# KorAP/Datok

Measured on AMD Instinct MI355X. Metric: input MB/s tokenized, tokenizer_de.matok, higher is better.
Workload: dtype u32 table cells, u8 symbol codes; 1 GPU; tokenizer_de.matok, 4096 equal-length 4096 B synthetic German docs per batch (BASELINE.json configs[1]); table_layout=matrix: state-major fused u32 cells, docs_per_gpu=4096, doc_bytes=4096, parallelism=documents sharded over 1 GPU(s), no data-path collective, batches_in_flight=3, inputs=one per batch in flight (generator seeds 2, 3, 4 on rank 0)

## Files before the change

### datok_amd/_lib.py

```python
import ctypes as C
import os
import subprocess

_HERE = os.path.dirname(os.path.abspath(__file__))
LIB_PATH = os.environ.get("DATOK_GPU_LIB") or os.path.join(_HERE, "libdatok_gpu.so")

OK, E_IO, E_FORMAT, E_NO_DEVICE, E_HIP, E_ARG, E_MODEL, E_CAPACITY, E_STATE, E_NOMEM = 0, -1, -2, -3, -4, -5, -6, -7, -8, -9
ST_WINDOW_OVERFLOW, ST_EMPTY_TEXT, ST_BAD_MODEL, ST_IRREGULAR, ST_STEP_LIMIT, ST_INTERNAL = 1, 2, 4, 8, 16, 32
ST_BAD_OFFSET = 64

EXPORTS = [
    "dtk_device_count", "dtk_set_device", "dtk_strerror", "dtk_last_hip_error",
    "dtk_model_load", "dtk_model_load_mem", "dtk_model_free", "dtk_model_type", "dtk_model_get_info",
    "dtk_model_info_mem",
    "dtk_batch_create", "dtk_batch_free", "dtk_batch_set_input", "dtk_batch_set_input_device",
    "dtk_batch_run", "dtk_batch_sync", "dtk_batch_stream", "dtk_batch_totals",
    "dtk_batch_set_profiling", "dtk_batch_stage_ms", "dtk_batch_set_chunking", "dtk_batch_set_warm_extend",
    "dtk_batch_result_device", "dtk_batch_result_host", "dtk_transduce", "dtk_free",
    "dtk_foma_to_matok", "dtk_foma_to_datok", "dtk_transduce_replay", "dtk_batch_render_device", "dtk_batch_render_host",
    "dtk_batch_status_host", "dtk_transduce_release", "dtk_transduce_result",
    "dtk_pipeline_create", "dtk_pipeline_free", "dtk_pipeline_set_chunking", "dtk_pipeline_run",
    "dtk_pinned_alloc", "dtk_pinned_free",
    "dtk_batch_set_result_fields", "dtk_batch_download_begin", "dtk_pipeline_set_result_fields",
    "dtk_batch_set_download_stream", "dtk_batch_download_stream", "dtk_batch_done", "dtk_batch_set_streams",
    "dtk_debug_configure",
    "dtk_multi_create", "dtk_multi_free", "dtk_multi_type", "dtk_multi_set_result_fields", "dtk_multi_set_chunking", "dtk_multi_run",
]


class ModelInfo(C.Structure):
    _fields_ = [("kind", C.c_int32), ("epsilon", C.c_int32), ("unknown", C.c_int32),
                ("identity", C.c_int32), ("final_state", C.c_int32), ("sigma_count", C.c_int32),
                ("state_count", C.c_uint32), ("array_len", C.c_uint64),
                ("n_eps_states", C.c_uint32), ("max_eps_chain", C.c_uint32),
                ("entry_bytes", C.c_uint32), ("device_bytes", C.c_uint64),
                ("unknown_used", C.c_uint32), ("dense_states", C.c_uint32),
                ("stream_codes", C.c_uint32)]


class Totals(C.Structure):
    _fields_ = [("n_docs", C.c_uint32), ("n_bytes", C.c_uint64), ("n_tokens", C.c_uint64),
                ("n_sent", C.c_uint64), ("n_texts", C.c_uint64), ("n_flagged", C.c_uint64),
                ("walk_steps", C.c_uint64), ("n_lanes", C.c_uint32), ("chunk_bytes", C.c_uint32),
                ("repair_rounds", C.c_uint32)]


class ResultView(C.Structure):
    _fields_ = [("tok_off", C.c_void_p), ("sent_off", C.c_void_p), ("text_off", C.c_void_p),
                ("tok_rstart", C.c_void_p), ("tok_rend", C.c_void_p),
                ("tok_bstart", C.c_void_p), ("tok_bend", C.c_void_p),
                ("sent", C.c_void_p), ("text_tok_end", C.c_void_p), ("text_sent_end", C.c_void_p),
                ("status", C.c_void_p), ("ev_bits", C.c_void_p), ("ev_words", C.c_uint64), ("doc_tail", C.c_void_p),
                ("n_exact", C.c_uint32), ("exact_doc", C.c_void_p), ("exact_off", C.c_void_p),
                ("calls", C.c_void_p), ("tok_r16", C.c_void_p)]


SLICE_FN = C.CFUNCTYPE(C.c_int, C.c_void_p, C.c_uint32, C.c_uint32, C.c_void_p)

# ... 75 lines not shown
    L.dtk_batch_download_stream.restype = vp
    L.dtk_pipeline_set_result_fields.argtypes = [vp, u32]
    L.dtk_transduce.argtypes = [vp, C.c_char_p, sz, u32, C.POINTER(vp), C.POINTER(sz), C.POINTER(u32)]
    L.dtk_transduce_replay.argtypes = L.dtk_transduce.argtypes
    L.dtk_transduce_release.restype = None
    L.dtk_transduce_result.argtypes = [vp, C.c_char_p, sz, u32, C.POINTER(ResultView)]
    L.dtk_batch_render_device.argtypes = [vp, u32, C.POINTER(RenderView)]
    L.dtk_batch_render_host.argtypes = [vp, u32, C.POINTER(RenderView)]
    L.dtk_batch_status_host.argtypes = [vp, vp, u32]
    L.dtk_foma_to_matok.argtypes = [vp, C.c_size_t, C.POINTER(vp), C.POINTER(C.c_size_t)]
    L.dtk_foma_to_matok.restype = C.c_int
    L.dtk_foma_to_datok.argtypes = [vp, C.c_size_t, C.POINTER(vp), C.POINTER(C.c_size_t)]
    L.dtk_foma_to_datok.restype = C.c_int
    L.dtk_free.argtypes = [vp]
    L.dtk_free.restype = None
    L.dtk_pipeline_create.argtypes = [u64, u32, u32, C.POINTER(vp)]
    L.dtk_pipeline_free.argtypes = [vp]
    L.dtk_pipeline_free.restype = None
    L.dtk_pipeline_set_chunking.argtypes = [vp, u32, u32]
    L.dtk_pipeline_run.argtypes = [vp, vp, vp, vp, u32, u32, SLICE_FN, vp]
    L.dtk_multi_create.argtypes = [C.c_char_p, C.POINTER(C.c_int), u32, u64, u32, u32, C.POINTER(vp)]
    L.dtk_multi_free.argtypes = [vp]
    L.dtk_multi_free.restype = None
    L.dtk_multi_type.argtypes = [vp]
    L.dtk_multi_type.restype = C.c_char_p
    L.dtk_multi_set_result_fields.argtypes = [vp, u32]
    L.dtk_multi_set_chunking.argtypes = [vp, u32, u32]
    L.dtk_multi_run.argtypes = [vp, vp, vp, u32, u32, SLICE_FN, vp]
    L.dtk_pinned_alloc.restype = vp
    L.dtk_pinned_alloc.argtypes = [sz]
    L.dtk_pinned_free.argtypes = [vp]
    L.dtk_pinned_free.restype = None
    L.dtk_debug_configure.argtypes = [C.c_char_p, C.c_char_p]
    for k, v in os.environ.items():
        if k.startswith("DATOK_") and k not in ("DATOK_GPU_LIB", "DATOK_GATHER_TIMEOUT"):
            L.dtk_debug_configure(k.encode(), v.encode())
    _lib = L
    return L


def check(code, what=""):
    if code != OK:
        raise DatokGpuError(code, what)
```

### datok_amd/csrc/dtk_batch.cpp

```cpp
#include <algorithm>
#include <cstdio>
#include <cstring>

#include "dtk_host.h"

int pin_fit(dtk_batch::PinBuf &pb, size_t n) {
  if (n <= pb.cap && pb.p) return DTK_OK;
  if (pb.p) HIP_TRY(hipHostFree(pb.p));
  pb.p = nullptr; pb.cap = 0;
  const size_t cap = std::max<size_t>(n + n / 4, 256);
  HIP_TRY(hipHostMalloc(&pb.p, cap, hipHostMallocDefault));
  pb.cap = cap;
  return DTK_OK;
}

static int alloc_outputs(dtk_batch *b, uint64_t tok, uint64_t sent, uint64_t text) {
  auto grow = [&](auto *&p, uint64_t n) -> int {
    if (p) HIP_TRY(hipFree(p));
    p = nullptr;
    HIP_TRY(hipMalloc((void **)&p, std::max<uint64_t>(n, 4) * 4));
    return DTK_OK;
  };
  int rc;
  if (tok > b->tok_cap) {
// ... 401 lines not shown
  b->repair_rounds = 0;
  hipStream_t s = b->stream;
  const bool prof = b->profiling;
#define STAGE(i) do { if (prof) HIP_TRY(hipEventRecord(b->ev[i], s)); } while (0)
  STAGE(0);
  bool fold_acc = false;
  size_t acc_bytes = 0;
  {
    const size_t nd = b->n_docs;
    uint8_t *q = b->d_acc;
    b->d_tok_off = b->d_csr; b->d_sent_off = b->d_csr + (nd + 1); b->d_text_off = b->d_csr + 2 * (nd + 1);
    b->d_totals = (uint64_t *)q; q += DTK_TOTALS_BYTES;
    b->d_tok_cnt = (uint64_t *)q; q += (nd + 1) * 8;
    b->d_sent_cnt = (uint64_t *)q; q += (nd + 1) * 8;
    b->d_text_cnt = (uint64_t *)q; q += (nd + 1) * 8;
    b->d_status = (uint32_t *)q; q += nd * 4;
    b->d_first_bad = (uint32_t *)q; q += nd * 4;
    b->d_fail_lane = (uint32_t *)q; q += nd * 4;
    b->d_doc_tail = (uint32_t *)q; q += nd * 4;
    const size_t acc_used = ((size_t)(q - b->d_acc) + 15) & ~(size_t)15;
    b->bit_words = (uint32_t)(((b->total + nd) / 32 + 8) & ~(uint64_t)3);
    const bool fold = b->total > 0;
    fold_acc = fold && b->acc_primed && acc_used / 16 < 0xFFFFFFFFull && !g_dbg.clear_kernel;
    if (!fold_acc) {
      if (dtk_launch_clear2(b->d_acc, acc_used, b->d_bits, fold ? 0 : (size_t)EVB_KINDS * b->bit_words * 4, s))
        return hip_fail(hipGetLastError(), "clear");
      b->acc_primed = true;
    }
    acc_bytes = acc_used;
  }
  STAGE(1);
  if (dtk_launch_symbolize(b->d_text, b->d_off, b->n_docs, b->total, &m->sig, b->d_sym,
                           b->d_text == b->d_text_own, b->d_blk_doc, (unsigned long long *)(b->d_totals + 6), b->d_rsbits,
                           b->d_bits, b->bit_words, fold_acc ? b->d_acc : nullptr, acc_bytes, ++b->epoch, s))
    return hip_fail(hipGetLastError(), "symbolize");
  STAGE(2);
  DtkWalkArgs w = walk_args(b);
  bool fix_in_scan = false;
  DtkSpecArgs sp_first{};
  if (b->chunk == 0) {
    STAGE(3); STAGE(4);
    if (dtk_launch_walk(&m->tab, &w, s)) return hip_fail(hipGetLastError(), "walk");
    STAGE(5); STAGE(6); STAGE(7);
  } else {
    DtkSpecArgs sp = spec_args(b, false);
    sp_first = sp;
    uint32_t *nb = (uint32_t *)(b->d_totals + 8);
    const bool split = g_dbg.split_start != 0 || sp.lds_words == 0;
    b->dev_rounds = g_dbg.dev_rounds >= 0 ? (uint32_t)g_dbg.dev_rounds : (b->expect_repairs ? 2u : 0u);
    if (b->dev_rounds > 3u) b->dev_rounds = 3u;
    fix_in_scan = b->n_docs <= 8192u && b->dev_rounds == 0;
#define SPEC(stage)                                                                               \
  do {                                                                                            \
    if (dtk_launch_spec(&m->tab, &w, &sp, stage, cmp_mask_of(m), b->d_redo, nb, s))               \
      return hip_fail(hipGetLastError(), "speculative walk");                                     \
  } while (0)
    if (split) {
      SPEC(0); STAGE(3); SPEC(1); STAGE(4); SPEC(2); STAGE(5); SPEC(3); STAGE(6);
    } else {
      STAGE(3); STAGE(4); SPEC(6); STAGE(5); SPEC(7); STAGE(6);
    }
    if (!fix_in_scan) SPEC(4);
    STAGE(7);
#undef SPEC
    for (uint32_t r = 0; r < b->dev_rounds; r++) {
      DtkSpecArgs rp = spec_args(b, true);
      rp.go = nb + r;
// ... 248 lines not shown
```

### datok_amd/csrc/dtk_host.h

```cpp
#pragma once
#include <hip/hip_runtime.h>

#include <string>
#include <type_traits>
#include <vector>

#include "../../include/datok_gpu.h"
#include "dtk_internal.h"

#pragma GCC visibility push(hidden)


int hip_fail(hipError_t e, const char *what);
#define HIP_TRY(call)                                   \
  do {                                                  \
    hipError_t e_ = (call);                             \
    if (e_ != hipSuccess) return hip_fail(e_, #call);   \
  } while (0)

struct DtkDebug {
  int sym16 = 0;
  int force_wide = 0;
  int file_columns = 0;
  int no_fused = 0;
  int wide_fused = 0;
  int no_dense = 0;
  int small_max = -1;
  int lds_bits = 1;
  int split_start = 0;
  int dev_rounds = -1;
  int compact_full = 0;
  int clear_kernel = 0;
  int round_limit = -1;
  int debug_repair = 0;
};
extern DtkDebug g_dbg;


struct dtk_model {
  int kind = 0;
  int epsilon = 0, unknown = 0, identity = 0, final_state = 0, sigma_count = 0;
  uint32_t state_count = 0;
  std::vector<uint16_t> col;
  uint32_t dense_states = 0;
  uint64_t array_len = 0;
  uint32_t n_eps_states = 0, max_eps_chain = 0, unknown_used = 0;
  uint64_t device_bytes = 0;
  int device = 0;
  bool host_only = false;
  std::vector<uint32_t> sigma_runes;
  std::vector<uint16_t> sigma_syms;
  uint16_t ascii[256];
  void *d_tab = nullptr;
  uint16_t *d_ascii = nullptr;
  uint32_t *d_runes = nullptr;
  uint16_t *d_syms = nullptr;
  void *d_codes = nullptr;
  DtkTableDev tab{};
  DtkSigmaDev sig{};
// ... 146 lines not shown
```

### datok_amd/csrc/dtk_internal.h

```cpp
#pragma once
#include <stddef.h>
#include <stdint.h>

#define DTK_FIRSTBIT 0x80000000u
#define DTK_SECONDBIT 0x40000000u
#define DTK_RESTBIT 0x3fffffffu
#define DTK_EOT 4u
#define DTK_WINDOW 1024u
#define DTK_WINDOW_BYTES 4104u

#define DTK_SYM_MASK 0x7FFu
#define DTK_SYM_MAX 2047u
#define DTK_SYM_W_SHIFT 11
#define DTK_SYM_CLS_SHIFT 14
#define DTK_SYM_WIDTH(e) (((uint32_t)(e) >> DTK_SYM_W_SHIFT) & 7u)
#define DTK_SYM_IS_START(e) (DTK_SYM_WIDTH(e) != 0u)
#define DTK_WIN 32u
#define DTK_WIN_ROW 36u
#define DTK_SYM_CONT 0xFFu
#ifndef DTK_WIN8
#define DTK_WIN8 32u
#endif
struct DtkSym {
  const void *base;
// ... 203 lines not shown
  const uint32_t *doc_ns;
  struct DtkSym sym;
  uint64_t *A, *P, *Q;
  uint64_t *blkA, *blkP, *blkQ;
  uint64_t *ns_off;
  uint64_t *tx_base, *tx_stream, *tx_pos, *tx_sent;
  uint64_t *out_off;
  uint8_t *out;
  uint64_t out_total;
};

#define DTK_TOHOST_MAX 14
struct DtkToHostArgs {
  const void *src[DTK_TOHOST_MAX];
  void *dst[DTK_TOHOST_MAX];
  uint64_t bytes[DTK_TOHOST_MAX];
  int32_t count_from[DTK_TOHOST_MAX];
  uint64_t cap[DTK_TOHOST_MAX];
  uint32_t n;
  const uint64_t *totals;
  const uint32_t *skip_if;
  uint64_t *done;
  uint64_t epoch;
};

#ifdef __cplusplus
extern "C" {
#endif
int dtk_launch_to_host(const struct DtkToHostArgs *args, void *stream);
int dtk_launch_pack_r16(const int32_t *rs, const int32_t *re, uint32_t *out, uint64_t n, void *stream);
int dtk_launch_symbolize(const uint8_t *text, const uint64_t *doc_off, uint32_t n_docs,
                         uint64_t total, const struct DtkSigmaDev *sig, void *sym, int padded,
                         const uint32_t *blk_doc, unsigned long long *n_invalid, uint32_t *rs_bits,
                         uint32_t *ev_bits, uint32_t bit_words, void *acc, uint64_t acc_bytes, uint64_t epoch, void *stream);
#ifndef DTK_SYM_BLOCK_BYTES
#define DTK_SYM_BLOCK_BYTES 4096u
#endif
int dtk_launch_walk(const struct DtkTableDev *tab, const struct DtkWalkArgs *args, void *stream);
int dtk_launch_spec(const struct DtkTableDev *tab, const struct DtkWalkArgs *args,
                    const struct DtkSpecArgs *spec, int stage, uint32_t cmp_mask, uint32_t *redo_out,
                    uint32_t *n_bad, void *stream);
int dtk_launch_spec_check(const struct DtkWalkArgs *args, const struct DtkSpecArgs *spec, int stage, uint32_t cmp_mask,
                          uint32_t *redo_out, uint32_t *n_bad, void *stream);
int dtk_launch_redo_clear(const struct DtkWalkArgs *args, const struct DtkSpecArgs *spec, void *stream);
int dtk_launch_compact(const struct DtkCompactArgs *args, uint32_t small_max, const uint32_t *big_docs, uint32_t n_big,
                       int which, void *stream);
int dtk_launch_exact(const struct DtkTableDev *tab, const struct DtkExactArgs *args, void *stream);
int dtk_launch_seg_prepare(const struct DtkCompactArgs *args, const uint32_t *doc_seg0, void *stream);
int dtk_launch_render(const struct DtkRenderArgs *args, int stage, void *stream);
uint32_t dtk_render_tiles(uint64_t n);
int dtk_launch_clear2(void *a, uint64_t a_bytes, void *b, uint64_t b_bytes, void *stream);
int dtk_launch_scan3(const uint64_t *ca, const uint64_t *cb, const uint64_t *cc, uint64_t *a, uint64_t *b,
                     uint64_t *c, uint32_t n_docs, uint64_t *totals, const uint32_t *status, uint64_t *ws,
                     const struct DtkSpecArgs *fix_spec, uint32_t *redo_out, uint32_t *n_bad, const uint32_t *skip_if,
                     void *stream);
#ifdef __cplusplus
}
#endif
```

### datok_amd/csrc/dtk_model.cpp

```cpp
#include <zlib.h>

#include <algorithm>
#include <cstdio>
#include <cstdlib>
#include <cstring>

#include "dtk_host.h"


static thread_local std::string g_hip_err;

int hip_fail(hipError_t e, const char *what) {
  g_hip_err = std::string(what) + ": " + hipGetErrorString(e);
  return e == hipErrorNoDevice || e == hipErrorInvalidDevice ? DTK_E_NO_DEVICE : DTK_E_HIP;
}

extern "C" const char *dtk_last_hip_error(void) { return g_hip_err.c_str(); }

extern "C" const char *dtk_strerror(int code) {
  switch (code) {
    case DTK_OK: return "ok";
    case DTK_E_IO: return "cannot open or read the tokenizer file";
    case DTK_E_FORMAT: return "not a gzip'd MATOK/DATOK file (magic, version or length)";
    case DTK_E_NO_DEVICE: return "no usable HIP device (this library has no CPU path)";
    case DTK_E_HIP: return "HIP runtime error (see dtk_last_hip_error)";
    case DTK_E_ARG: return "invalid argument";
    case DTK_E_MODEL: return "model outside device limits (symbols >= 2048, special ids out of range, epsilon cycle)";
    case DTK_E_CAPACITY: return "batch exceeds the capacity it was created with";
    case DTK_E_STATE: return "call out of order";
    case DTK_E_NOMEM: return "out of host memory";
    default: return "unknown error";
  }
}

extern "C" int dtk_device_count(void) {
  int n = 0;
  if (hipGetDeviceCount(&n) != hipSuccess) return 0;
  return n;
}

extern "C" int dtk_set_device(int device) {
  HIP_TRY(hipSetDevice(device));
  return DTK_OK;
}

DtkDebug g_dbg;

extern "C" int dtk_debug_configure(const char *key, const char *value) {
  if (!key) return DTK_E_ARG;
  const int v = value ? atoi(value) : 1;
  const struct { const char *name; int *field; bool flag; } tab[] = {
      {"SYM16", &g_dbg.sym16, true}, {"FORCE_WIDE", &g_dbg.force_wide, true}, {"FILE_COLUMNS", &g_dbg.file_columns, true},
      {"NO_FUSED", &g_dbg.no_fused, true}, {"WIDE_FUSED", &g_dbg.wide_fused, true}, {"NO_DENSE", &g_dbg.no_dense, true}, {"SMALL_MAX", &g_dbg.small_max, false},
      {"LDS_BITS", &g_dbg.lds_bits, false}, {"SPLIT_START", &g_dbg.split_start, false}, {"DEV_ROUNDS", &g_dbg.dev_rounds, false},
      {"COMPACT_FULL", &g_dbg.compact_full, true}, {"CLEAR_KERNEL", &g_dbg.clear_kernel, true},
      {"ROUND_LIMIT", &g_dbg.round_limit, false}, {"DEBUG_REPAIR", &g_dbg.debug_repair, true}};
  if (strncmp(key, "DATOK_", 6) == 0) key += 6;
  for (const auto &e : tab)
    if (strcmp(key, e.name) == 0) {
      *e.field = e.flag ? ((value && value[0] == '0' && value[1] == 0) ? 0 : 1) : v;
      return DTK_OK;
    }
  return DTK_E_ARG;
}


int go_decode_host(const uint8_t *p, size_t n, uint32_t *r) {
  *r = 0xFFFD;
  if (n == 0) return 0;
  uint32_t b0 = p[0];
  if (b0 < 0x80) { *r = b0; return 1; }
  if (b0 < 0xC2 || b0 > 0xF4) return 1;
  if (b0 < 0xE0) {
    if (n < 2 || (p[1] & 0xC0) != 0x80) return 1;
    *r = ((b0 & 0x1F) << 6) | (p[1] & 0x3F);
    return 2;
  }
  if (b0 < 0xF0) {
    uint32_t lo = b0 == 0xE0 ? 0xA0 : 0x80, hi = b0 == 0xED ? 0x9F : 0xBF;
    if (n < 3 || p[1] < lo || p[1] > hi || (p[2] & 0xC0) != 0x80) return 1;
    *r = ((b0 & 0x0F) << 12) | ((uint32_t)(p[1] & 0x3F) << 6) | (p[2] & 0x3F);
    return 3;
  }
  uint32_t lo = b0 == 0xF0 ? 0x90 : 0x80, hi = b0 == 0xF4 ? 0x8F : 0xBF;
  if (n < 4 || p[1] < lo || p[1] > hi || (p[2] & 0xC0) != 0x80 || (p[3] & 0xC0) != 0x80) return 1;
  *r = ((b0 & 0x07) << 18) | ((uint32_t)(p[1] & 0x3F) << 12) | ((uint32_t)(p[2] & 0x3F) << 6) | (p[3] & 0x3F);
// ... 508 lines not shown
```

### datok_amd/csrc/dtk_symbolize.hip

```cpp
#include "dtk_device.h"


__device__ __forceinline__ uint32_t go_width(uint32_t b0, uint32_t b1, uint32_t b2, uint32_t b3, uint32_t avail) {
  const uint32_t c1 = (b1 & 0xC0u) == 0x80u, c2 = (b2 & 0xC0u) == 0x80u, c3 = (b3 & 0xC0u) == 0x80u;
  const uint32_t two = (uint32_t)(b0 - 0xC2u < 0x1Eu) & (uint32_t)(avail >= 2u) & c1;
  const uint32_t lo3 = b0 == 0xE0u ? 0xA0u : 0x80u, hi3 = b0 == 0xEDu ? 0x9Fu : 0xBFu;
  const uint32_t three = (uint32_t)((b0 & 0xF0u) == 0xE0u) & (uint32_t)(avail >= 3u) & (uint32_t)(b1 >= lo3) &
                         (uint32_t)(b1 <= hi3) & c2;
  const uint32_t lo4 = b0 == 0xF0u ? 0x90u : 0x80u, hi4 = b0 == 0xF4u ? 0x8Fu : 0xBFu;
  const uint32_t four = (uint32_t)(b0 - 0xF0u <= 4u) & (uint32_t)(avail >= 4u) & (uint32_t)(b1 >= lo4) &
                        (uint32_t)(b1 <= hi4) & c2 & c3;
  return 1u + two + 2u * three + 3u * four;
}


#define SYM_BLOCK_BYTES DTK_SYM_BLOCK_BYTES
#define SYM_TILE 512u
#define SYM_SIG_LDS 64u
#define SYM_HALF 1024u
#define SYM_THREADS (WAVE * (SYM_BLOCK_BYTES / SYM_HALF))
#define SYM_DOFF (SYM_BLOCK_BYTES / 16u)

template <bool ALIGNED4, bool SYM8>
__global__ __launch_bounds__(SYM_THREADS) void k_symbolize(const uint8_t *__restrict__ text,
                                                    const uint64_t *__restrict__ doc_off,
                                                    uint32_t n_docs, uint64_t total, DtkSigmaDev sig,
                                                    void *__restrict__ sym_,
                                                    const uint32_t *__restrict__ blk_doc,
                                                    unsigned long long *__restrict__ n_invalid,
                                                    uint32_t *__restrict__ rs_bits,
                                                    uint32_t *__restrict__ ev_bits, uint32_t bit_words,
                                                    uint4 *__restrict__ acc, uint32_t acc16,
                                                    unsigned long long epoch) {
  if (acc) {
    const uint4 z = make_uint4(0u, 0u, 0u, 0u);
    for (uint32_t i = blockIdx.x * SYM_THREADS + threadIdx.x; i < acc16; i += gridDim.x * SYM_THREADS) {
      if (i == 3u) reinterpret_cast<unsigned long long *>(acc)[7] = 0ull;
      else acc[i] = z;
    }
  }
  uint16_t *__restrict__ sym = static_cast<uint16_t *>(sym_);
  uint8_t *__restrict__ sym8 = static_cast<uint8_t *>(sym_);
  __shared__ uint32_t s_rs[SYM_BLOCK_BYTES / 32];
  __shared__ uint16_t lut[128];
  __shared__ uint16_t lat[256];
  __shared__ uint32_t s_runes[SYM_SIG_LDS];
  __shared__ uint16_t s_syms[SYM_SIG_LDS];
  __shared__ uint32_t s_txt[SYM_BLOCK_BYTES / 4 + 4];
  __shared__ uint16_t s_qs[SYM_BLOCK_BYTES / SYM_HALF][SYM_HALF];
  __shared__ uint64_t s_doff[SYM_DOFF];
  const uint32_t tid = threadIdx.x, lane = tid & (WAVE - 1u), half = tid >> 6;
  uint16_t *s_q = s_qs[half];
  const bool sig_lds = sig.n_runes <= SYM_SIG_LDS;
  for (uint32_t i = tid; i < SYM_BLOCK_BYTES / 32; i += SYM_THREADS) s_rs[i] = 0;
  for (uint32_t i = tid; i < 256u; i += SYM_THREADS) {
    if (SYM8) {
      lat[i] = sig.code_lt256[i];
      if (sig_lds && i < sig.n_runes) { s_runes[i] = sig.runes[i]; s_syms[i] = sig.code_runes[i]; }
    } else {
      const uint32_t e = (sig.ascii[i] & DTK_SYM_MASK) | (i == DTK_EOT ? (1u << DTK_SYM_CLS_SHIFT) : 0u);
      lat[i] = (uint16_t)e;
      if (i < 128u) lut[i] = (uint16_t)(e | (1u << DTK_SYM_W_SHIFT));
      if (sig_lds && i < sig.n_runes) { s_runes[i] = sig.runes[i]; s_syms[i] = sig.syms[i]; }
    }
  }
  const uint64_t block_start = (uint64_t)blockIdx.x * SYM_BLOCK_BYTES;
  const uint32_t n_here = (uint32_t)min((uint64_t)SYM_BLOCK_BYTES, total - block_start);
  const uint32_t d_lo = blk_doc[blockIdx.x];
  const uint32_t d_hi = min(blk_doc[blockIdx.x + 1], n_docs - 1);
  const uint32_t n_off = d_hi - d_lo + 2u;
  if (n_off <= SYM_DOFF && tid < n_off) s_doff[tid] = doc_off[d_lo + tid];
  {
    auto load4 = [&](uint64_t g) -> uint32_t {
      if (ALIGNED4) return g < total ? *reinterpret_cast<const uint32_t *>(text + g) : 0u;
      uint32_t x = 0;
      for (int k = 0; k < 4; k++)
        if (g + k < total) x |= (uint32_t)text[g + k] << (8 * k);
      return x;
    };
    uint32_t v[SYM_BLOCK_BYTES / 4 / SYM_THREADS];
#pragma unroll
    for (uint32_t r = 0; r < SYM_BLOCK_BYTES / 4 / SYM_THREADS; r++) v[r] = load4(block_start + (r * SYM_THREADS + tid) * 4u);
    uint32_t halo = 0;
    if (tid == 0 && block_start >= 4) halo = load4(block_start - 4);
    if (tid == 1) halo = load4(block_start + SYM_BLOCK_BYTES);
#pragma unroll
    for (uint32_t r = 0; r < SYM_BLOCK_BYTES / 4 / SYM_THREADS; r++) s_txt[1 + r * SYM_THREADS + tid] = v[r];
    if (tid == 0) s_txt[0] = halo;
    if (tid == 1) s_txt[1 + SYM_BLOCK_BYTES / 4] = halo;
  }
  __syncthreads();
  const uint8_t *__restrict__ sb = reinterpret_cast<const uint8_t *>(s_txt) + 4;

  const uint64_t lo_start = doc_off[d_lo], lo_end = doc_off[d_lo + 1];
  if (ev_bits) {
    const uint64_t ga = block_start + d_lo, gb = block_start + n_here + d_hi + 1u;
    const uint32_t wa = blockIdx.x == 0 ? 0u : (uint32_t)(ga >> 5);
    uint32_t wb = (uint32_t)((gb + 31u) >> 5);
    if (wb > bit_words || blockIdx.x == gridDim.x - 1) wb = bit_words;
    for (uint32_t w = wa + tid; w < wb; w += SYM_THREADS)
#pragma unroll
      for (uint32_t k = 0; k < EVB_KINDS; k++) ev_bits[(size_t)k * bit_words + w] = 0u;
  }
  const bool sym16 = ((reinterpret_cast<uintptr_t>(sym_) + (SYM8 ? 1ull : 2ull) * block_start) & (SYM8 ? 7u : 15u)) == 0;

  if (half * SYM_HALF < n_here) {
    uint32_t qn = 0;
    auto light = [&](auto full_tag, uint32_t it) {
      constexpr bool FULL = decltype(full_tag)::value;
      const uint32_t i0 = half * SYM_HALF + it * SYM_TILE + lane * 8u;
      const uint32_t w0 = s_txt[1 + (i0 >> 2)], w1 = s_txt[2 + (i0 >> 2)];
      uint32_t left = 8u;
      if (!FULL) left = i0 < n_here ? (n_here - i0 >= 8u ? 8u : n_here - i0) : 0u;
      if (SYM8) {
        if (FULL || (left == 8u && sym16)) {
          *reinterpret_cast<uint2 *>(sym8 + block_start + i0) = make_uint2(w0, w1);
        } else {
          for (uint32_t j = 0; j < left; j++) sym8[block_start + i0 + j] = (uint8_t)((j < 4u ? w0 >> (8u * j) : w1 >> (8u * j - 32u)));
        }
      } else {
        const uint32_t e0 = lut[w0 & 0x7Fu], e1 = lut[(w0 >> 8) & 0x7Fu];
        const uint32_t e2 = lut[(w0 >> 16) & 0x7Fu], e3 = lut[(w0 >> 24) & 0x7Fu];
        const uint32_t e4 = lut[w1 & 0x7Fu], e5 = lut[(w1 >> 8) & 0x7Fu];
        const uint32_t e6 = lut[(w1 >> 16) & 0x7Fu], e7 = lut[(w1 >> 24) & 0x7Fu];
        if (FULL || (left == 8u && sym16)) {
          *reinterpret_cast<uint4 *>(sym + block_start + i0) =
              make_uint4(e0 | (e1 << 16), e2 | (e3 << 16), e4 | (e5 << 16), e6 | (e7 << 16));
        } else {
          const uint32_t o[8] = {e0, e1, e2, e3, e4, e5, e6, e7};
          for (uint32_t j = 0; j < left; j++) sym[block_start + i0 + j] = (uint16_t)o[j];
        }
      }
      auto nib = [](uint32_t x) { return ((x >> 7) & 1u) | ((x >> 14) & 2u) | ((x >> 21) & 4u) | ((x >> 28) & 8u); };
      const uint32_t valid = FULL ? 0xFFu : ((1u << left) - 1u);
      const uint32_t rare = (nib(w0 & 0x80808080u) | (nib(w1 & 0x80808080u) << 4)) & valid;
      const uint32_t asc = ~rare & valid;
// ... 75 lines not shown
            const int m = (l + h) >> 1;
            const uint32_t r = sig_lds ? s_runes[m] : sig.runes[m];
            if (r == rune) {
              if (SYM8)
                a_cls = wd == 1u ? (uint32_t)sig.code_fffd1 : (sig_lds ? (uint32_t)s_syms[m] : (uint32_t)sig.code_runes[m]);
              else
                a_cls = ((sig_lds ? (uint32_t)s_syms[m] : (uint32_t)sig.syms[m]) & DTK_SYM_MASK) |
                        (2u << DTK_SYM_CLS_SHIFT);
              break;
            }
            if (r < rune) l = m + 1; else h = m - 1;
          }
        }
        if (SYM8) sym8[g] = (uint8_t)(start ? a_cls : DTK_SYM_CONT);
        else sym[g] = (uint16_t)(a_cls | (start ? wd << DTK_SYM_W_SHIFT : 0u));
        if (start) atomicOr(&s_rs[pos >> 5], 1u << (pos & 31u));
        bad = start && wd == 1u;
      }
      if (__ballot(bad) != 0ull && lane == 0 &&
          __hip_atomic_load(n_invalid, __ATOMIC_RELAXED, __HIP_MEMORY_SCOPE_AGENT) != epoch)
        atomicMax(n_invalid, epoch);
    }
  }
  __syncthreads();
  for (uint32_t i = tid; i < SYM_BLOCK_BYTES / 32; i += SYM_THREADS)
    if (i * 32u < n_here) rs_bits[(block_start >> 5) + i] = s_rs[i];
}


extern "C" int dtk_launch_symbolize(const uint8_t *text, const uint64_t *doc_off, uint32_t n_docs,
                                    uint64_t total, const DtkSigmaDev *sig, void *sym, int padded,
                                    const uint32_t *blk_doc, unsigned long long *n_invalid, uint32_t *rs_bits,
                                    uint32_t *ev_bits, uint32_t bit_words, void *acc, uint64_t acc_bytes,
                                    uint64_t epoch, void *stream) {
  if (total == 0 || n_docs == 0) return 0;
  const uint32_t blocks = (uint32_t)((total + SYM_BLOCK_BYTES - 1) / SYM_BLOCK_BYTES);
  const bool al4 = (((uintptr_t)text) & 3u) == 0 && (padded || (total & 3u) == 0);
  auto go = [&](auto k) {
    hipLaunchKernelGGL(k, dim3(blocks), dim3(SYM_THREADS), 0, (hipStream_t)stream, text, doc_off, n_docs,
                       total, *sig, sym, blk_doc, n_invalid, rs_bits, ev_bits, bit_words, (uint4 *)acc, (uint32_t)(acc_bytes / 16),
                       (unsigned long long)epoch);
  };
  if (sig->n_codes) { if (al4) go(k_symbolize<true, true>); else go(k_symbolize<false, true>); }
  else { if (al4) go(k_symbolize<true, false>); else go(k_symbolize<false, false>); }
  return (int)hipGetLastError();
}
```

### include/datok_gpu.h

```cpp
#ifndef DATOK_GPU_H
#define DATOK_GPU_H

#include <stddef.h>
#include <stdint.h>

#ifdef __cplusplus
extern "C" {
#endif

enum {
  DTK_OK = 0,
  DTK_E_IO = -1,
  DTK_E_FORMAT = -2,
  DTK_E_NO_DEVICE = -3,
  DTK_E_HIP = -4,
  DTK_E_ARG = -5,
  DTK_E_MODEL = -6,
  DTK_E_CAPACITY = -7,
  DTK_E_STATE = -8,
  DTK_E_NOMEM = -9
};

enum {
  DTK_TOKENS = 1,
  DTK_SENTENCES = 2,
  DTK_TOKEN_POS = 4,
  DTK_SENTENCE_POS = 8,
  DTK_NEWLINE_AFTER_EOT = 16,
  DTK_SIMPLE = 3,
  DTK_OFFSETS_ONLY = 256,
  DTK_NO_BYTE_OFFSETS = 512,
  DTK_NO_RUNE_OFFSETS = 1024
};

enum {
  DTK_ST_WINDOW_OVERFLOW = 1,
  DTK_ST_EMPTY_TEXT = 2,
  DTK_ST_BAD_MODEL = 4,
  DTK_ST_IRREGULAR = 8,
  DTK_ST_STEP_LIMIT = 16,
  DTK_ST_INTERNAL = 32,
  DTK_ST_BAD_OFFSET = 64
};

typedef struct dtk_model dtk_model;
typedef struct dtk_batch dtk_batch;

int dtk_device_count(void);
int dtk_set_device(int device);
const char *dtk_strerror(int code);
const char *dtk_last_hip_error(void);

int dtk_debug_configure(const char *key, const char *value);

int dtk_model_load(const char *path, dtk_model **out);
int dtk_model_load_mem(const void *gz_bytes, size_t n, dtk_model **out);
void dtk_model_free(dtk_model *m);
int dtk_foma_to_matok(const void *gz_bytes, size_t n, void **out, size_t *out_n);
int dtk_foma_to_datok(const void *gz_bytes, size_t n, void **out, size_t *out_n);
const char *dtk_model_type(const dtk_model *m);

typedef struct {
  int32_t kind;
  int32_t epsilon, unknown, identity, final_state, sigma_count;
  uint32_t state_count;
  uint64_t array_len;
  uint32_t n_eps_states;
  uint32_t max_eps_chain;
  uint32_t entry_bytes;
  uint64_t device_bytes;
  uint32_t unknown_used;
  uint32_t dense_states;
  uint32_t stream_codes;
} dtk_model_info;
int dtk_model_get_info(const dtk_model *m, dtk_model_info *out);
int dtk_model_info_mem(const void *gz_bytes, size_t n, dtk_model_info *out);

int dtk_batch_create(uint64_t max_bytes, uint32_t max_docs, dtk_batch **out);
void dtk_batch_free(dtk_batch *b);

int dtk_batch_set_input(dtk_batch *b, const uint8_t *text, const uint64_t *doc_off, uint32_t n_docs);
int dtk_batch_set_input_device(dtk_batch *b, const void *d_text, const void *d_doc_off,
                               uint32_t n_docs, uint64_t total_bytes);

int dtk_batch_set_chunking(dtk_batch *b, uint32_t chunk_bytes, uint32_t warm_bytes);

// ... 117 lines not shown
```

Baseline: 171,200 MB/s.

## Add register-only SWAR fast path for UTF-8 symbolization of full blocks

Result: faster. 182,800 MB/s (median of 6 runs) (+6.8%).

```diff
diff --git a/datok_amd/_lib.py b/datok_amd/_lib.py
--- a/datok_amd/_lib.py
+++ b/datok_amd/_lib.py
@@ -23,7 +23,7 @@
     "dtk_pinned_alloc", "dtk_pinned_free",
     "dtk_batch_set_result_fields", "dtk_batch_download_begin", "dtk_pipeline_set_result_fields",
     "dtk_batch_set_download_stream", "dtk_batch_download_stream", "dtk_batch_done", "dtk_batch_set_streams",
-    "dtk_debug_configure",
+    "dtk_debug_configure", "dtk_debug_symbolize_lanes",
     "dtk_multi_create", "dtk_multi_free", "dtk_multi_type", "dtk_multi_set_result_fields", "dtk_multi_set_chunking", "dtk_multi_run",
 ]
 
@@ -165,6 +165,7 @@
     L.dtk_pinned_free.argtypes = [vp]
     L.dtk_pinned_free.restype = None
     L.dtk_debug_configure.argtypes = [C.c_char_p, C.c_char_p]
+    L.dtk_debug_symbolize_lanes.argtypes = [vp, u64, vp, u32, vp, vp, vp, u32, vp, vp, vp, vp]
     for k, v in os.environ.items():
         if k.startswith("DATOK_") and k not in ("DATOK_GPU_LIB", "DATOK_GATHER_TIMEOUT"):
             L.dtk_debug_configure(k.encode(), v.encode())
diff --git a/datok_amd/csrc/dtk_batch.cpp b/datok_amd/csrc/dtk_batch.cpp
--- a/datok_amd/csrc/dtk_batch.cpp
+++ b/datok_amd/csrc/dtk_batch.cpp
@@ -457,7 +457,8 @@
   STAGE(1);
   if (dtk_launch_symbolize(b->d_text, b->d_off, b->n_docs, b->total, &m->sig, b->d_sym,
                            b->d_text == b->d_text_own, b->d_blk_doc, (unsigned long long *)(b->d_totals + 6), b->d_rsbits,
-                           b->d_bits, b->bit_words, fold_acc ? b->d_acc : nullptr, acc_bytes, ++b->epoch, s))
+                           b->d_bits, b->bit_words, fold_acc ? b->d_acc : nullptr, acc_bytes, ++b->epoch,
+                           !g_dbg.no_fast_sym, s))
     return hip_fail(hipGetLastError(), "symbolize");
   STAGE(2);
   DtkWalkArgs w = walk_args(b);
diff --git a/datok_amd/csrc/dtk_host.h b/datok_amd/csrc/dtk_host.h
--- a/datok_amd/csrc/dtk_host.h
+++ b/datok_amd/csrc/dtk_host.h
@@ -25,6 +25,7 @@
   int no_fused = 0;
   int wide_fused = 0;
   int no_dense = 0;
+  int no_fast_sym = 0;
   int small_max = -1;
   int lds_bits = 1;
   int split_start = 0;
diff --git a/datok_amd/csrc/dtk_internal.h b/datok_amd/csrc/dtk_internal.h
--- a/datok_amd/csrc/dtk_internal.h
+++ b/datok_amd/csrc/dtk_internal.h
@@ -259,7 +259,8 @@
 int dtk_launch_symbolize(const uint8_t *text, const uint64_t *doc_off, uint32_t n_docs,
                          uint64_t total, const struct DtkSigmaDev *sig, void *sym, int padded,
                          const uint32_t *blk_doc, unsigned long long *n_invalid, uint32_t *rs_bits,
-                         uint32_t *ev_bits, uint32_t bit_words, void *acc, uint64_t acc_bytes, uint64_t epoch, void *stream);
+                         uint32_t *ev_bits, uint32_t bit_words, void *acc, uint64_t acc_bytes, uint64_t epoch, int fast,
+                         void *stream);
 #ifndef DTK_SYM_BLOCK_BYTES
 #define DTK_SYM_BLOCK_BYTES 4096u
 #endif
diff --git a/datok_amd/csrc/dtk_model.cpp b/datok_amd/csrc/dtk_model.cpp
--- a/datok_amd/csrc/dtk_model.cpp
+++ b/datok_amd/csrc/dtk_model.cpp
@@ -51,7 +51,7 @@
   const int v = value ? atoi(value) : 1;
   const struct { const char *name; int *field; bool flag; } tab[] = {
       {"SYM16", &g_dbg.sym16, true}, {"FORCE_WIDE", &g_dbg.force_wide, true}, {"FILE_COLUMNS", &g_dbg.file_columns, true},
-      {"NO_FUSED", &g_dbg.no_fused, true}, {"WIDE_FUSED", &g_dbg.wide_fused, true}, {"NO_DENSE", &g_dbg.no_dense, true}, {"SMALL_MAX", &g_dbg.small_max, false},
+      {"NO_FUSED", &g_dbg.no_fused, true}, {"WIDE_FUSED", &g_dbg.wide_fused, true}, {"NO_DENSE", &g_dbg.no_dense, true}, {"NO_FAST_SYM", &g_dbg.no_fast_sym, true}, {"SMALL_MAX", &g_dbg.small_max, false},
       {"LDS_BITS", &g_dbg.lds_bits, false}, {"SPLIT_START", &g_dbg.split_start, false}, {"DEV_ROUNDS", &g_dbg.dev_rounds, false},
       {"COMPACT_FULL", &g_dbg.compact_full, true}, {"CLEAR_KERNEL", &g_dbg.clear_kernel, true},
       {"ROUND_LIMIT", &g_dbg.round_limit, false}, {"DEBUG_REPAIR", &g_dbg.debug_repair, true}};
diff --git a/datok_amd/csrc/dtk_symbolize.hip b/datok_amd/csrc/dtk_symbolize.hip
--- a/datok_amd/csrc/dtk_symbolize.hip
+++ b/datok_amd/csrc/dtk_symbolize.hip
@@ -1,4 +1,5 @@
 #include "dtk_device.h"
+#include "dtk_symbolize_lane.h"
 
 
 __device__ __forceinline__ uint32_t go_width(uint32_t b0, uint32_t b1, uint32_t b2, uint32_t b3, uint32_t avail) {
@@ -21,8 +22,8 @@
 #define SYM_THREADS (WAVE * (SYM_BLOCK_BYTES / SYM_HALF))
 #define SYM_DOFF (SYM_BLOCK_BYTES / 16u)
 
-template <bool ALIGNED4, bool SYM8>
-__global__ __launch_bounds__(SYM_THREADS) void k_symbolize(const uint8_t *__restrict__ text,
+template <bool ALIGNED4, bool SYM8, bool FAST>
+__global__ __launch_bounds__(SYM_THREADS, FAST ? 8 : 1) void k_symbolize(const uint8_t *__restrict__ text,
                                                     const uint64_t *__restrict__ doc_off,
                                                     uint32_t n_docs, uint64_t total, DtkSigmaDev sig,
                                                     void *__restrict__ sym_,
@@ -70,7 +71,66 @@
   const uint32_t d_hi = min(blk_doc[blockIdx.x + 1], n_docs - 1);
   const uint32_t n_off = d_hi - d_lo + 2u;
   if (n_off <= SYM_DOFF && tid < n_off) s_doff[tid] = doc_off[d_lo + tid];
-  {
+  auto clear_events = [&]() {
+    const uint64_t ga = block_start + d_lo, gb = block_start + n_here + d_hi + 1u;
+    const uint32_t wa = blockIdx.x == 0 ? 0u : (uint32_t)(ga >> 5);
+    uint32_t wb = (uint32_t)((gb + 31u) >> 5);
+    if (wb > bit_words || blockIdx.x == gridDim.x - 1) wb = bit_words;
+    for (uint32_t w = wa + tid; w < wb; w += SYM_THREADS)
+#pragma unroll
+      for (uint32_t k = 0; k < EVB_KINDS; k++) ev_bits[(size_t)k * bit_words + w] = 0u;
+  };
+  bool staged = false;
+  if constexpr (FAST) {
+    static_assert(ALIGNED4 && SYM8 && SYM_THREADS * DTK_SYM_LANE_BYTES == SYM_BLOCK_BYTES, "one lane per 16 bytes of the block");
+    __shared__ uint32_t s_vote[SYM_THREADS / WAVE];
+    if (n_here == SYM_BLOCK_BYTES) {
+      const uint32_t i0 = tid * DTK_SYM_LANE_BYTES;
+      const uint64_t g = block_start + i0;
+      uint64_t starts[DTK_SYM_FAST_DOCS];
+#pragma unroll
+      for (uint32_t i = 0; i < DTK_SYM_FAST_DOCS; i++) starts[i] = doc_off[min(d_lo + i, n_docs)];
+      const uint64_t g_next = g + DTK_SYM_LANE_BYTES;
+      const bool has_prev = g >= 4u, has_next = g_next < total;
+      const uint64_t a_halo = lane == 0u ? (has_prev ? g - 4u : g) : (lane == WAVE - 1u && has_next ? g_next : g);
+      const uint4 v = *reinterpret_cast<const uint4 *>(text + g);
+      const uint32_t halo = *reinterpret_cast<const uint32_t *>(text + a_halo);
+      if (ev_bits) clear_events();
+      const uint32_t fw0 = v.x, fw1 = v.y, fw2 = v.z, fw3 = v.w;
+      const uint32_t up = (uint32_t)__shfl_up((int)fw3, 1), dn = (uint32_t)__shfl_down((int)fw0, 1);
+      const uint32_t tail = total - g_next >= 4u ? 0xFFFFFFFFu : (1u << (8u * ((uint32_t)(total - g_next) & 3u))) - 1u;
+      const uint32_t fprev = lane == 0u ? (has_prev ? halo : 0u) : up;
+      const uint32_t fnext = lane == WAVE - 1u ? (has_next ? halo & tail : 0u) : dn;
+      DtkSymLane fl = dtk_sym_classify(fw0, fw1, fw2, fw3, fprev, fnext, DTK_SYM_LANE_BYTES);
+      uint32_t ok = fl.ok;
+#pragma unroll
+      for (uint32_t i = 0; i < DTK_SYM_FAST_DOCS; i++)
+        ok &= dtk_sym_doc_start_bad(fl.cross, i0, dtk_sym_doc_rel(starts[i], block_start)) ^ 1u;
+      if (dtk_sym_docs_beyond(starts[DTK_SYM_FAST_DOCS - 1u], block_start, d_lo, n_docs)) ok = 0u;
+      const uint32_t declined = __ballot(ok == 0u) != 0ull;
+      if (lane == 0u) s_vote[half] = declined;
+      __syncthreads();
+      if ((s_vote[0] | s_vote[1] | s_vote[2] | s_vote[3]) == 0u) {
+        const uint32_t ident234 = (uint32_t)sig.code_ident[2] | ((uint32_t)sig.code_ident[3] << 8) | ((uint32_t)sig.code_ident[4] << 16);
+        for (uint32_t m = fl.lead; __builtin_amdgcn_ballot_w64(m != 0u) != 0ull; m &= m - 1u)
+          if (m) {
+            const uint32_t j = (uint32_t)__builtin_ctz(m);
+            const uint32_t c = sig_lds ? dtk_sym_lead_code(fw0, fw1, fw2, fw3, fnext, j, lat, s_runes, s_syms, sig.n_runes, ident234)
+                                       : dtk_sym_lead_code(fw0, fw1, fw2, fw3, fnext, j, lat, sig.runes, sig.code_runes, sig.n_runes, ident234);
+            fl = dtk_sym_patch(fl, j, c);
+          }
+        *reinterpret_cast<uint4 *>(sym8 + g) = make_uint4(fl.o0, fl.o1, fl.o2, fl.o3);
+        const uint32_t other = (uint32_t)__builtin_amdgcn_update_dpp(0, (int)fl.rs, 0xB1, 0xF, 0xF, true);
+        if ((tid & 1u) == 0u) rs_bits[(block_start >> 5) + (tid >> 1)] = fl.rs | (other << 16);
+        return;
+      }
+      s_txt[1u + tid * 4u] = fw0; s_txt[2u + tid * 4u] = fw1; s_txt[3u + tid * 4u] = fw2; s_txt[4u + tid * 4u] = fw3;
+      if (tid == 0) s_txt[0] = fprev;
+      if (tid == SYM_THREADS - 1u) s_txt[1 + SYM_BLOCK_BYTES / 4] = fnext;
+      staged = true;
+    }
+  }
+  if (!staged) {
     auto load4 = [&](uint64_t g) -> uint32_t {
       if (ALIGNED4) return g < total ? *reinterpret_cast<const uint32_t *>(text + g) : 0u;
       uint32_t x = 0;
@@ -93,15 +153,7 @@
   const uint8_t *__restrict__ sb = reinterpret_cast<const uint8_t *>(s_txt) + 4;
 
   const uint64_t lo_start = doc_off[d_lo], lo_end = doc_off[d_lo + 1];
-  if (ev_bits) {
-    const uint64_t ga = block_start + d_lo, gb = block_start + n_here + d_hi + 1u;
-    const uint32_t wa = blockIdx.x == 0 ? 0u : (uint32_t)(ga >> 5);
-    uint32_t wb = (uint32_t)((gb + 31u) >> 5);
-    if (wb > bit_words || blockIdx.x == gridDim.x - 1) wb = bit_words;
-    for (uint32_t w = wa + tid; w < wb; w += SYM_THREADS)
-#pragma unroll
-      for (uint32_t k = 0; k < EVB_KINDS; k++) ev_bits[(size_t)k * bit_words + w] = 0u;
-  }
+  if (!staged && ev_bits) clear_events();
   const bool sym16 = ((reinterpret_cast<uintptr_t>(sym_) + (SYM8 ? 1ull : 2ull) * block_start) & (SYM8 ? 7u : 15u)) == 0;
 
   if (half * SYM_HALF < n_here) {
@@ -243,7 +295,7 @@
                                     uint64_t total, const DtkSigmaDev *sig, void *sym, int padded,
                                     const uint32_t *blk_doc, unsigned long long *n_invalid, uint32_t *rs_bits,
                                     uint32_t *ev_bits, uint32_t bit_words, void *acc, uint64_t acc_bytes,
-                                    uint64_t epoch, void *stream) {
+                                    uint64_t epoch, int fast, void *stream) {
   if (total == 0 || n_docs == 0) return 0;
   const uint32_t blocks = (uint32_t)((total + SYM_BLOCK_BYTES - 1) / SYM_BLOCK_BYTES);
   const bool al4 = (((uintptr_t)text) & 3u) == 0 && (padded || (total & 3u) == 0);
@@ -252,7 +304,13 @@
                        total, *sig, sym, blk_doc, n_invalid, rs_bits, ev_bits, bit_words, (uint4 *)acc, (uint32_t)(acc_bytes / 16),
                        (unsigned long long)epoch);
   };
-  if (sig->n_codes) { if (al4) go(k_symbolize<true, true>); else go(k_symbolize<false, true>); }
-  else { if (al4) go(k_symbolize<true, false>); else go(k_symbolize<false, false>); }
+  const bool al16 = ((((uintptr_t)text) | ((uintptr_t)sym)) & 15u) == 0;
+  if (sig->n_codes) {
+    if (al4 && al16 && fast) go(k_symbolize<true, true, true>);
+    else if (al4) go(k_symbolize<true, true, false>);
+    else go(k_symbolize<false, true, false>);
+  } else {
+    if (al4) go(k_symbolize<true, false, false>); else go(k_symbolize<false, false, false>);
+  }
   return (int)hipGetLastError();
 }
diff --git a/datok_amd/csrc/dtk_symbolize_host.cpp b/datok_amd/csrc/dtk_symbolize_host.cpp
--- /dev/null
+++ b/datok_amd/csrc/dtk_symbolize_host.cpp
@@ -0,0 +1,67 @@
+#include <hip/hip_runtime.h>
+#include <string.h>
+
+#include "../../include/datok_gpu.h"
+#include "dtk_symbolize_lane.h"
+
+namespace {
+
+uint32_t dword_at(const uint8_t *text, uint64_t total, int64_t g) {
+  uint32_t x = 0;
+  for (int k = 0; k < 4; k++)
+    if (g + k >= 0 && (uint64_t)(g + k) < total) x |= (uint32_t)text[g + k] << (8 * k);
+  return x;
+}
+
+}
+
+extern "C" int dtk_debug_symbolize_lanes(const uint8_t *text, uint64_t total, const uint64_t *doc_off, uint32_t n_docs,
+                                         const uint8_t *code_lt256, const uint32_t *runes, const uint8_t *rune_codes,
+                                         uint32_t n_runes, const uint8_t *code_ident, uint8_t *codes, uint32_t *rs_bits,
+                                         uint8_t *eligible) {
+  if (!text || !doc_off || n_docs == 0 || !code_lt256 || !code_ident || !codes || !rs_bits || !eligible ||
+      (n_runes && (!runes || !rune_codes)))
+    return DTK_E_ARG;
+  const uint32_t lanes = DTK_SYM_BLOCK_BYTES / DTK_SYM_LANE_BYTES;
+  const uint32_t ident234 = (uint32_t)code_ident[2] | ((uint32_t)code_ident[3] << 8) | ((uint32_t)code_ident[4] << 16);
+  const uint64_t blocks = (total + DTK_SYM_BLOCK_BYTES - 1) / DTK_SYM_BLOCK_BYTES;
+  uint32_t d_lo = 0;
+  for (uint64_t b = 0; b < blocks; b++) {
+    const uint64_t block_start = b * DTK_SYM_BLOCK_BYTES;
+    const uint32_t n_here = (uint32_t)(total - block_start < DTK_SYM_BLOCK_BYTES ? total - block_start : DTK_SYM_BLOCK_BYTES);
+    while (d_lo + 1 < n_docs && doc_off[d_lo + 1] <= block_start) d_lo++;
+    uint32_t rel[DTK_SYM_FAST_DOCS];
+    uint64_t last = 0;
+    for (uint32_t i = 0; i < DTK_SYM_FAST_DOCS; i++) {
+      last = doc_off[d_lo + i < n_docs ? d_lo + i : n_docs];
+      rel[i] = dtk_sym_doc_rel(last, block_start);
+    }
+    uint32_t ok = dtk_sym_docs_beyond(last, block_start, d_lo, n_docs) ^ 1u;
+    DtkSymLane L[DTK_SYM_BLOCK_BYTES / DTK_SYM_LANE_BYTES];
+    uint32_t w[DTK_SYM_BLOCK_BYTES / DTK_SYM_LANE_BYTES][4], next[DTK_SYM_BLOCK_BYTES / DTK_SYM_LANE_BYTES];
+    for (uint32_t t = 0; t < lanes; t++) {
+      const uint64_t g = block_start + t * DTK_SYM_LANE_BYTES;
+      const uint32_t i0 = t * DTK_SYM_LANE_BYTES;
+      const uint32_t nvalid = i0 < n_here ? (n_here - i0 < DTK_SYM_LANE_BYTES ? n_here - i0 : DTK_SYM_LANE_BYTES) : 0u;
+      for (int k = 0; k < 4; k++) w[t][k] = dword_at(text, total, (int64_t)g + 4 * k);
+      next[t] = dword_at(text, total, (int64_t)g + 16);
+      L[t] = dtk_sym_classify(w[t][0], w[t][1], w[t][2], w[t][3], dword_at(text, total, (int64_t)g - 4), next[t], nvalid);
+      ok &= L[t].ok;
+      for (uint32_t i = 0; i < DTK_SYM_FAST_DOCS; i++) ok &= dtk_sym_doc_start_bad(L[t].cross, i0, rel[i]) ^ 1u;
+    }
+    eligible[b] = (uint8_t)ok;
+    if (!ok) continue;
+    for (uint32_t t = 0; t < lanes && t * DTK_SYM_LANE_BYTES < n_here; t++) {
+      for (uint32_t m = L[t].lead; m; m &= m - 1u) {
+        const uint32_t j = (uint32_t)__builtin_ctz(m);
+        L[t] = dtk_sym_patch(L[t], j, dtk_sym_lead_code(w[t][0], w[t][1], w[t][2], w[t][3], next[t], j, code_lt256, runes, rune_codes, n_runes, ident234));
+      }
+      const uint64_t g = block_start + t * DTK_SYM_LANE_BYTES;
+      for (uint32_t j = 0; j < DTK_SYM_LANE_BYTES && g + j < total; j++) codes[g + j] = (uint8_t)dtk_sym_out_byte(L[t], j);
+      uint32_t &word = rs_bits[g >> 5];
+      const uint32_t sh = (uint32_t)(g & 31u);
+      word = (word & ~(0xFFFFu << sh)) | (L[t].rs << sh);
+    }
+  }
+  return DTK_OK;
+}
diff --git a/datok_amd/csrc/dtk_symbolize_lane.h b/datok_amd/csrc/dtk_symbolize_lane.h
--- /dev/null
+++ b/datok_amd/csrc/dtk_symbolize_lane.h
@@ -0,0 +1,134 @@
+#pragma once
+#include <stdint.h>
+
+#include "dtk_internal.h"
+
+#ifdef __HIP__
+#define DTK_LANE_FN __attribute__((host)) __attribute__((device)) inline __attribute__((always_inline))
+#else
+#define DTK_LANE_FN static inline
+#endif
+
+#define DTK_SYM_H 0x80808080u
+#define DTK_SYM_LANE_BYTES 16u
+#define DTK_SYM_FAST_DOCS 8u
+
+static_assert(DTK_SYM_CONT == 0xFFu, "continuation bytes are turned into their code by an OR");
+
+struct DtkSymPlanes {
+  uint32_t cont;
+  uint32_t a1, a2, a3;
+  uint32_t bad;
+};
+
+DTK_LANE_FN DtkSymPlanes dtk_sym_planes(uint32_t x) {
+  const uint32_t t6 = x << 1, t5 = x << 2, t4 = x << 3, t3 = x << 4, t2 = x << 5, t1 = x << 6, t0 = x << 7;
+  DtkSymPlanes p;
+  p.cont = x & ~t6;
+  p.a1 = x & t6;
+  p.a2 = p.a1 & t5;
+  p.a3 = p.a2 & t4;
+  const uint32_t l3 = p.a2 & ~t4, o10 = t1 | t0;
+  const uint32_t c01 = p.a1 & ~(t5 | t4 | t3 | t2 | t1);
+  const uint32_t f = p.a3 & (t3 | t2 | ~o10);
+  const uint32_t e0 = l3 & ~(t3 | t2 | o10);
+  const uint32_t ed = l3 & t3 & t2 & ~t1 & t0;
+  p.bad = c01 | f | e0 | ed;
+  return p;
+}
+
+DTK_LANE_FN uint32_t dtk_sym_pack4(uint32_t f) { return (((f >> 7) & 0x01010101u) * 0x01020408u) >> 24; }
+DTK_LANE_FN uint32_t dtk_sym_up(uint32_t hi, uint32_t lo, uint32_t n) { return (hi << (8u * n)) | (lo >> (32u - 8u * n)); }
+
+struct DtkSymLane {
+  uint32_t o0, o1, o2, o3;
+  uint32_t rs;
+  uint32_t lead;
+  uint32_t cross;
+  uint32_t ok;
+};
+
+DTK_LANE_FN DtkSymLane dtk_sym_classify(uint32_t w0, uint32_t w1, uint32_t w2, uint32_t w3, uint32_t prev, uint32_t next,
+                                        uint32_t nvalid) {
+  DtkSymLane L;
+  const uint32_t valid = nvalid >= 16u ? 0xFFFFu : (1u << nvalid) - 1u;
+  if (((w0 | w1 | w2 | w3 | prev) & DTK_SYM_H) == 0u) {
+    L.o0 = w0; L.o1 = w1; L.o2 = w2; L.o3 = w3;
+    L.rs = valid; L.lead = 0u; L.cross = 0u; L.ok = 1u;
+    return L;
+  }
+  const DtkSymPlanes pp = dtk_sym_planes(prev), p0 = dtk_sym_planes(w0), p1 = dtk_sym_planes(w1),
+                     p2 = dtk_sym_planes(w2), p3 = dtk_sym_planes(w3);
+  uint32_t bad = pp.bad | p0.bad | p1.bad | p2.bad | p3.bad;
+  bad |= ((pp.a1 << 8) | (pp.a2 << 16) | (pp.a3 << 24)) & ~pp.cont;
+  bad |= (dtk_sym_up(p0.a1, pp.a1, 1) | dtk_sym_up(p0.a2, pp.a2, 2) | dtk_sym_up(p0.a3, pp.a3, 3)) ^ p0.cont;
+  bad |= (dtk_sym_up(p1.a1, p0.a1, 1) | dtk_sym_up(p1.a2, p0.a2, 2) | dtk_sym_up(p1.a3, p0.a3, 3)) ^ p1.cont;
+  bad |= (dtk_sym_up(p2.a1, p1.a1, 1) | dtk_sym_up(p2.a2, p1.a2, 2) | dtk_sym_up(p2.a3, p1.a3, 3)) ^ p2.cont;
+  bad |= (dtk_sym_up(p3.a1, p2.a1, 1) | dtk_sym_up(p3.a2, p2.a2, 2) | dtk_sym_up(p3.a3, p2.a3, 3)) ^ p3.cont;
+  const uint32_t reach = (p3.a1 >> 24) | (p3.a2 >> 16) | (p3.a3 >> 8);
+  bad |= reach & ~(next & ~(next << 1));
+  L.ok = (bad & DTK_SYM_H) == 0u;
+  const uint32_t cont = dtk_sym_pack4(p0.cont) | (dtk_sym_pack4(p1.cont) << 4) | (dtk_sym_pack4(p2.cont) << 8) |
+                        (dtk_sym_pack4(p3.cont) << 12);
+  L.lead = dtk_sym_pack4(p0.a1) | (dtk_sym_pack4(p1.a1) << 4) | (dtk_sym_pack4(p2.a1) << 8) | (dtk_sym_pack4(p3.a1) << 12);
+  L.rs = ~cont & valid;
+  L.cross = dtk_sym_pack4(pp.cont) | (cont << 4) | (dtk_sym_pack4(reach) << 20);
+  const uint32_t c0 = p0.cont & DTK_SYM_H, c1 = p1.cont & DTK_SYM_H, c2 = p2.cont & DTK_SYM_H, c3 = p3.cont & DTK_SYM_H;
+  L.o0 = w0 | c0 | (c0 - (c0 >> 7));
+  L.o1 = w1 | c1 | (c1 - (c1 >> 7));
+  L.o2 = w2 | c2 | (c2 - (c2 >> 7));
+  L.o3 = w3 | c3 | (c3 - (c3 >> 7));
+  return L;
+}
+
+DTK_LANE_FN uint32_t dtk_sym_doc_rel(uint64_t s, uint64_t block_start) {
+  const uint64_t r = s + 4u - block_start;
+  const uint32_t hi = (uint32_t)(r >> 32), lo = (uint32_t)r;
+  return (hi | (lo >> 16)) == 0u ? lo : 0xFFFFFFFFu;
+}
+DTK_LANE_FN uint32_t dtk_sym_doc_start_bad(uint32_t cross, uint32_t i0, uint32_t rel) {
+  const uint32_t d = rel - i0;
+  return d < 23u ? (cross >> d) & 1u : 0u;
+}
+
+DTK_LANE_FN uint32_t dtk_sym_docs_beyond(uint64_t last, uint64_t block_start, uint32_t d_lo, uint32_t n_docs) {
+  return last < block_start + DTK_SYM_BLOCK_BYTES + 3u && d_lo + DTK_SYM_FAST_DOCS - 1u < n_docs;
+}
+
+template <class LT, class RC>
+DTK_LANE_FN uint32_t dtk_sym_lead_code(uint32_t w0, uint32_t w1, uint32_t w2, uint32_t w3, uint32_t next, uint32_t j, const LT *lt256,
+                                       const uint32_t *runes, const RC *rune_codes, uint32_t n_runes, uint32_t ident234) {
+  const uint32_t k = j >> 2;
+  const uint32_t lo = k == 0u ? w0 : (k == 1u ? w1 : (k == 2u ? w2 : w3));
+  const uint32_t hi = k == 0u ? w1 : (k == 1u ? w2 : (k == 2u ? w3 : next));
+  const uint32_t x = (uint32_t)((((uint64_t)hi << 32) | lo) >> (8u * (j & 3u)));
+  const uint32_t b0 = x & 0xFFu, b1 = (x >> 8) & 0x3Fu, b2 = (x >> 16) & 0x3Fu, b3 = x >> 24 & 0x3Fu;
+  const uint32_t wd = b0 >= 0xF0u ? 4u : (b0 >= 0xE0u ? 3u : 2u);
+  const uint32_t r2 = ((b0 & 0x1Fu) << 6) | b1, r3 = ((b0 & 0x0Fu) << 12) | (b1 << 6) | b2;
+  const uint32_t r4 = ((b0 & 0x07u) << 18) | (b1 << 12) | (b2 << 6) | b3;
+  const uint32_t rune = wd == 2u ? r2 : (wd == 3u ? r3 : r4);
+  if (rune < 256u) return (uint32_t)lt256[rune];
+  uint32_t code = (ident234 >> (8u * (wd - 2u))) & 0xFFu;
+  int l = 0, h = (int)n_runes - 1;
+  while (l <= h) {
+    const int m = (l + h) >> 1;
+    const uint32_t r = runes[m];
+    if (r == rune) { code = (uint32_t)rune_codes[m]; break; }
+    if (r < rune) l = m + 1; else h = m - 1;
+  }
+  return code;
+}
+
+DTK_LANE_FN DtkSymLane dtk_sym_patch(DtkSymLane L, uint32_t j, uint32_t code) {
+  const uint32_t sh = 8u * (j & 3u), m = 0xFFu << sh, v = code << sh, k = j >> 2;
+  L.o0 = k == 0u ? (L.o0 & ~m) | v : L.o0;
+  L.o1 = k == 1u ? (L.o1 & ~m) | v : L.o1;
+  L.o2 = k == 2u ? (L.o2 & ~m) | v : L.o2;
+  L.o3 = k == 3u ? (L.o3 & ~m) | v : L.o3;
+  return L;
+}
+
+DTK_LANE_FN uint32_t dtk_sym_out_byte(const DtkSymLane &L, uint32_t j) {
+  const uint32_t k = j >> 2, x = k == 0u ? L.o0 : (k == 1u ? L.o1 : (k == 2u ? L.o2 : L.o3));
+  return (x >> (8u * (j & 3u))) & 0xFFu;
+}
diff --git a/include/datok_gpu.h b/include/datok_gpu.h
--- a/include/datok_gpu.h
+++ b/include/datok_gpu.h
@@ -52,6 +52,10 @@
 const char *dtk_last_hip_error(void);
 
 int dtk_debug_configure(const char *key, const char *value);
+int dtk_debug_symbolize_lanes(const uint8_t *text, uint64_t total, const uint64_t *doc_off, uint32_t n_docs,
+                              const uint8_t *code_lt256, const uint32_t *runes, const uint8_t *rune_codes,
+                              uint32_t n_runes, const uint8_t *code_ident, uint8_t *codes, uint32_t *rs_bits,
+                              uint8_t *eligible);
 
 int dtk_model_load(const char *path, dtk_model **out);
 int dtk_model_load_mem(const void *gz_bytes, size_t n, dtk_model **out);
```
